# humanoid-path-planner/hpp-fcl

Hardware: AMD Instinct MI355X
Metric: narrow-phase queries/s (collision+distance) (higher is better)
Workload: dtype f32; 1 GPU; cfg3_convex32_distance_nesterov; request=distance, gather=none

## Files before the change

hpp-fcl_amd/csrc/hfcl_dev.hpp:

```cpp
#pragma once
#include <hip/hip_runtime.h>

#include <cstdint>
#include <cstring>
#include <type_traits>

#include "../../include/hppfcl_amd.h"
#include "hfcl_bvh.hpp"
#include "hfcl_bvh_shape.hpp"
#include "hfcl_epa_pool.hpp"
#include "hfcl_pair.hpp"

using namespace hfcl;

#ifndef HFCL_WPE_GJK_W2
#define HFCL_WPE_GJK_W2 2
#endif
#ifndef HFCL_WPE_GJK
#define HFCL_WPE_GJK 3
#endif
#ifndef HFCL_WPE_GJK64
#define HFCL_WPE_GJK64 2
#endif
#ifndef HFCL_WPE_PRIM
#define HFCL_WPE_PRIM 2
#endif
#ifndef HFCL_WPE_EPA32
#define HFCL_WPE_EPA32 2
#endif
#ifndef HFCL_WPE_EPA64
#define HFCL_WPE_EPA64 1
#endif
#ifndef HFCL_WPE_BVH
#define HFCL_WPE_BVH 1
#endif

enum { B_CLOSED = 0, B_PRIM = 1, B_CC = 2, B_PC = 3, B_CP = 4, B_BVH = 5, B_UNSUPPORTED = 6, B_LARGE = 7, B_BVHSHAPE = 8, B_TRI = 9, B_COUNT = 10 };
constexpr int B_CURVED0 = B_COUNT + 4;
constexpr int CTR_SHAPE_TICKET = 2 * B_COUNT + 4, CTR_SHAPE_DEFER = 2 * B_COUNT + 5;
constexpr int CTR_DIST_SUSP = 2 * B_COUNT + 6;
constexpr int CTR_SHAPE_DIST_SUSP = 2 * B_COUNT + 7;
constexpr int CTR_DIST_TICKET = 2 * B_COUNT + 8;
constexpr int CTR_SHAPE_DIST_TICKET = 2 * B_COUNT + 9;
constexpr int CTR_EPA_CC_OVER = 2 * B_COUNT + 10;
constexpr int CTR_SHAPE_FINISH_OVER = 2 * B_COUNT + 11;
constexpr int CTR_SHAPE_DEFER_MARK = 2 * B_COUNT + 13;
constexpr int CTR_DIST_RERUN = 2 * B_COUNT + 14, CTR_SHAPE_DIST_RERUN = 2 * B_COUNT + 15;
constexpr int N_COUNTERS = 2 * B_COUNT + 16;
constexpr int EPA_POOL_CTR0 = (N_COUNTERS + EPA_POOL_STRIDE_WORDS - 1) / EPA_POOL_STRIDE_WORDS * EPA_POOL_STRIDE_WORDS;
constexpr int N_COUNTER_WORDS = EPA_POOL_CTR0 + EPA_POOL_K * EPA_POOL_STRIDE_WORDS;

constexpr int K_CONVEX_LARGE = 21;

__host__ __device__ inline int bucket_of(int k1, int k2, bool distance_mode = false) {
  if (distance_mode && (k1 == K_TRIANGLE || k2 == K_TRIANGLE)) return B_UNSUPPORTED;
  const bool large = (k1 == K_CONVEX_LARGE) || (k2 == K_CONVEX_LARGE);
  if (k1 == K_CONVEX_LARGE) k1 = K_CONVEX;
  if (k2 == K_CONVEX_LARGE) k2 = K_CONVEX;
  if ((k1 == K_BVH) != (k2 == K_BVH)) {
    const int o = (k1 == K_BVH) ? k2 : k1;
    return (kind_is_prim(o) || o == K_CONVEX || kind_is_flat(o)) ? B_BVHSHAPE : B_UNSUPPORTED;
  }
  if ((k1 == K_TRIANGLE || k2 == K_TRIANGLE) && !kind_is_flat(k1) && !kind_is_flat(k2)) {
    const int o = (k1 == K_TRIANGLE) ? k2 : k1;
    return (o == K_TRIANGLE || kind_is_prim(o) || o == K_CONVEX) ? B_TRI : B_UNSUPPORTED;
  }
  const int c = pair_class(k1, k2);
  if (large && c == CLS_CONVEX) return B_LARGE;
  if (c == CLS_CLOSED) return B_CLOSED;
  if (c == CLS_PRIM_GJK) return B_PRIM;
  if (c == CLS_BVH) return B_BVH;
  if (c == CLS_CONVEX) {
    if (k1 == K_CONVEX && k2 == K_CONVEX) return B_CC;
    return (k1 == K_CONVEX) ? B_CP : B_PC;
  }
  return B_UNSUPPORTED;
}

template <typename T>
struct NbrEntry;
template <> struct alignas(16) NbrEntry<float> { float x, y, z; uint32_t id; };
template <> struct alignas(32) NbrEntry<double> { double x, y, z; uint32_t id; uint32_t pad_; };

template <typename T>
struct LibView {
  const DShape<T>* shapes;
  const T* verts;
  const uint8_t* kinds;
  uint32_t n_shapes;
  const uint32_t* graph_base;
  const uint32_t* graph_off;
  const NbrEntry<T>* graph_ent;
  uint32_t climb_min;
};
static constexpr uint32_t HFCL_NO_GRAPH = 0xFFFFFFFFu;
#ifndef HFCL_CLIMB_MIN
#define HFCL_CLIMB_MIN 512u
#endif
static constexpr int HFCL_WARM_STARTS = 14;
template <typename T>
struct HullGraph {
  const uint32_t* off;
  const NbrEntry<T>* ent;
};
template <typename T>
__device__ __forceinline__ HullGraph<T> hull_graph(const LibView<T>& lib, uint32_t shape_id, uint32_t num_points) {
  HullGraph<T> g{nullptr, nullptr};
  if (lib.graph_base == nullptr || num_points < lib.climb_min) return g;
  const uint32_t base = lib.graph_base[shape_id];
  if (base == HFCL_NO_GRAPH) return g;
  g.off = lib.graph_off + base;
  g.ent = lib.graph_ent;
  return g;
}

template <typename T> struct IO;
template <> struct IO<double> {
  const double* tf1;
  const double* tf2;
  hfcl_result* out;
  const hfcl_guess* gin;
  hfcl_guess* gout;
};
template <> struct IO<float> {
  const float* tf1;
  const float* tf2;
  hfcl_result_f32* out;
  const hfcl_guess* gin;
  hfcl_guess* gout;
};

template <typename T> using EpaItem = EpaSeed<T>;

struct Work {
  const uint32_t* shape1;
  const uint32_t* shape2;
  uint32_t n;
  uint32_t* lists;
  uint32_t* counts;
  void* epa_queue;
  void* epa_queue2;
  void* epa_v0;
  void* epa_resume;
  uint32_t resume_cap;
  void* shape_defer;
  uint32_t shape_defer_cap;
  uint32_t* shape_finish_over;
  void* shape_oq;
  void* epa_ready;
  void* epa_ready_g;
  uint32_t* epa_cc_over;
  uint32_t cc_resume_base, cc_resume_cap;
};
__host__ __device__ inline bool curved_pair(int k1, int k2) {
  return k1 == K_ELLIPSOID || k1 == K_CONE || k1 == K_CYLINDER || k2 == K_ELLIPSOID || k2 == K_CONE || k2 == K_CYLINDER;
}
struct BucketList {
  const uint32_t* base;
  uint32_t n, c0, cnt;
  __device__ __forceinline__ uint32_t operator[](uint32_t i) const { return i < c0 ? base[i] : base[n - 1u - (i - c0)]; }
};
__device__ __forceinline__ BucketList bucket_list(const Work& wk, int b) {
  const uint32_t c0 = wk.counts[b];
  return BucketList{wk.lists + size_t(b) * wk.n, wk.n, c0, c0 + wk.counts[B_CURVED0 + b]};
}
constexpr int32_t EPA_RESUME_FLAG = 0x100;
constexpr int32_t EPA_RESUME_SMALL = 0x200;

__device__ __forceinline__ Pose<double> load_pose(const double* base, uint32_t i) { return pose_from_abi<double>(base + 12 * size_t(i)); }
__device__ __forceinline__ void put_record(hfcl_result* dst, const hfcl_result& r) { *dst = r; }
__device__ __forceinline__ Pose<float> load_pose(const float* base, uint32_t i) { return pose_from_quat<float>(base + 7 * size_t(i)); }

__device__ __forceinline__ void store_record(const IO<double>& io, uint32_t pair, const PairOut<double>& o, bool contact,
                                             int nc) {
  hfcl_result r;
  r.distance = o.distance;
  r.normal[0] = o.normal.x; r.normal[1] = o.normal.y; r.normal[2] = o.normal.z;
  r.p1[0] = o.p1.x; r.p1[1] = o.p1.y; r.p1[2] = o.p1.z;
  r.p2[0] = o.p2.x; r.p2[1] = o.p2.y; r.p2[2] = o.p2.z;
  r.b1 = -1;
  r.b2 = -1;
  r.status = pack_status(o.gjk_status, o.epa_status, contact, o.gjk_iters, o.epa_iters);
  r.num_contacts = nc;
  put_record(&io.out[pair], r);
}
__device__ __forceinline__ void store_record(const IO<float>& io, uint32_t pair, const PairOut<float>& o, bool contact,
                                             int) {
  hfcl_result_f32 r;
  r.distance = o.distance;
  r.p1[0] = o.p1.x; r.p1[1] = o.p1.y; r.p1[2] = o.p1.z;
  r.p2[0] = o.p2.x; r.p2[1] = o.p2.y; r.p2[2] = o.p2.z;
  r.normal[0] = o.normal.x; r.normal[1] = o.normal.y; r.normal[2] = o.normal.z;
  r.status = pack_status(o.gjk_status, o.epa_status, contact, o.gjk_iters, o.epa_iters);
  io.out[pair] = r;
}
template <typename T>
__device__ __forceinline__ void write_out(const IO<T>& io, const QParams<T>& q, uint32_t pair, PairOut<T> o) {
  int nc;
  const bool contact = apply_query_semantics(q, o, nc);
  store_record(io, pair, o, contact, nc);
}

__device__ __forceinline__ void store_bvh_record(const IO<double>& io, uint32_t pair, const PairOut<double>& o, uint32_t nc,
                                                 int b1, int b2, bool overflow) {
  hfcl_result r;
  r.distance = o.distance;
  r.normal[0] = o.normal.x; r.normal[1] = o.normal.y; r.normal[2] = o.normal.z;
  r.p1[0] = o.p1.x; r.p1[1] = o.p1.y; r.p1[2] = o.p1.z;
  r.p2[0] = o.p2.x; r.p2[1] = o.p2.y; r.p2[2] = o.p2.z;
  r.b1 = b1;
  r.b2 = b2;
  r.status = (nc ? 128u : 0u) | (overflow ? 0xC0000000u : 0u);
  r.num_contacts = int(nc & 0x7FFFFFFFu);
  io.out[pair] = r;
}
__device__ __forceinline__ void store_bvh_record(const IO<float>& io, uint32_t pair, const PairOut<float>& o, uint32_t nc,
                                                 int, int, bool overflow) {
  hfcl_result_f32 r;
  r.distance = o.distance;
  r.p1[0] = o.p1.x; r.p1[1] = o.p1.y; r.p1[2] = o.p1.z;
  r.p2[0] = o.p2.x; r.p2[1] = o.p2.y; r.p2[2] = o.p2.z;
  r.normal[0] = o.normal.x; r.normal[1] = o.normal.y; r.normal[2] = o.normal.z;
  r.status = (nc ? 128u : 0u) | (overflow ? 0xC0000000u : 0u);
  io.out[pair] = r;
}

__device__ __forceinline__ void store_witness(const IO<double>& io, uint32_t pair, const V3<double>& p1, const V3<double>& p2, const V3<double>& n) {
  hfcl_result* r = &io.out[pair];
  r->normal[0] = n.x; r->normal[1] = n.y; r->normal[2] = n.z;
  r->p1[0] = p1.x; r->p1[1] = p1.y; r->p1[2] = p1.z;
  r->p2[0] = p2.x; r->p2[1] = p2.y; r->p2[2] = p2.z;
}
__device__ __forceinline__ void store_witness(const IO<float>& io, uint32_t pair, const V3<float>& p1, const V3<float>& p2, const V3<float>& n) {
  hfcl_result_f32* r = &io.out[pair];
  r->p1[0] = p1.x; r->p1[1] = p1.y; r->p1[2] = p1.z;
  r->p2[0] = p2.x; r->p2[1] = p2.y; r->p2[2] = p2.z;
  r->normal[0] = n.x; r->normal[1] = n.y; r->normal[2] = n.z;
}
template <typename T>
__device__ __forceinline__ void load_witness(const IO<T>& io, uint32_t pair, V3<T>& p1, V3<T>& p2, V3<T>& n) {
  const auto* r = &io.out[pair];
  n = mk<T>(T(r->normal[0]), T(r->normal[1]), T(r->normal[2]));
  p1 = mk<T>(T(r->p1[0]), T(r->p1[1]), T(r->p1[2]));
  p2 = mk<T>(T(r->p2[0]), T(r->p2[1]), T(r->p2[2]));
}
__device__ __forceinline__ void store_bvh_record_head(const IO<double>& io, uint32_t pair, double distance, uint32_t nc, int b1, int b2, bool overflow) {
  hfcl_result* r = &io.out[pair];
  r->distance = distance;
  r->b1 = b1;
  r->b2 = b2;
  r->status = (nc ? 128u : 0u) | (overflow ? 0xC0000000u : 0u);
  r->num_contacts = int(nc & 0x7FFFFFFFu);
}
__device__ __forceinline__ void store_bvh_record_head(const IO<float>& io, uint32_t pair, float distance, uint32_t nc, int, int, bool overflow) {
  hfcl_result_f32* r = &io.out[pair];
  r->distance = distance;
  r->status = (nc ? 128u : 0u) | (overflow ? 0xC0000000u : 0u);
}

template <typename T>
__device__ __forceinline__ void write_guess(const IO<T>&, uint32_t, const V3<T>&, int, int) {}
template <>
__device__ __forceinline__ void write_guess<double>(const IO<double>& io, uint32_t pair, const V3<double>& g, int h0, int h1) {
  if (io.gout) {
    hfcl_guess r;
    r.gjk_guess[0] = g.x; r.gjk_guess[1] = g.y; r.gjk_guess[2] = g.z;
    r.support_guess[0] = h0;
    r.support_guess[1] = h1;
    io.gout[pair] = r;
  }
}

template <typename T>
__device__ __forceinline__ V3<T> initial_guess(const IO<T>& io, const QParams<T>& q, uint32_t pair) {
  if (q.guess_mode == HFCL_GUESS_CACHED || q.guess_mode == HFCL_GUESS_BOUNDING_VOLUME)
    return mk<T>(q.guess[0], q.guess[1], q.guess[2]);
  return mk<T>(T(1), T(0), T(0));
}
template <>
__device__ __forceinline__ V3<double> initial_guess<double>(const IO<double>& io, const QParams<double>& q, uint32_t pair) {
  if (q.guess_mode == HFCL_GUESS_CACHED) {
    if (io.gin) return mk<double>(io.gin[pair].gjk_guess[0], io.gin[pair].gjk_guess[1], io.gin[pair].gjk_guess[2]);
    return mk<double>(q.guess[0], q.guess[1], q.guess[2]);
  }
  if (q.guess_mode == HFCL_GUESS_BOUNDING_VOLUME) return mk<double>(q.guess[0], q.guess[1], q.guess[2]);
  return mk<double>(1.0, 0.0, 0.0);
}
template <int CTRL, class X>
__device__ __forceinline__ X dpp_move(X v) {
  static_assert(sizeof(X) % 4 == 0, "32-bit words");
  int w[sizeof(X) / 4];
  __builtin_memcpy(w, &v, sizeof(X));
#pragma unroll
  for (int i = 0; i < int(sizeof(X) / 4); ++i) w[i] = __builtin_amdgcn_update_dpp(w[i], w[i], CTRL, 0xF, 0xF, false);
  X r;
  __builtin_memcpy(&r, w, sizeof(X));
  return r;
}
template <int W, int M, class X>
__device__ __forceinline__ X group_exchange(X v) {
  static_assert(M >= 1 && M < W, "stage of a W-lane butterfly");
  if constexpr (M == 1) return dpp_move<0xB1>(v);
  else if constexpr (M == 2) return dpp_move<0x4E>(v);
  else if constexpr (M == 4) return dpp_move<0x141>(v);
  else if constexpr (M == 8) return dpp_move<0x140>(v);
  else {
    int w[sizeof(X) / 4];
    __builtin_memcpy(w, &v, sizeof(X));
#pragma unroll
    for (int i = 0; i < int(sizeof(X) / 4); ++i) w[i] = __shfl_xor(w[i], M, W);
    X r;
    __builtin_memcpy(&r, w, sizeof(X));
    return r;
  }
}

constexpr int HULL_MAX = 32;
constexpr int HULL_LARGE_MAX = 1 << 16;

template <typename T, int W>
struct HullRegs {
  static constexpr int VPL = (HULL_MAX + W - 1) / W;
  V3<T> v[VPL];

  __device__ __forceinline__ void load(const T* verts, uint32_t n, int lig) {
#pragma unroll
    for (int k = 0; k < VPL; ++k) {
      uint32_t idx = uint32_t(lig * VPL + k);
      idx = idx < n ? idx : 0u;
      const T* p = verts + 3 * size_t(idx);
      v[k] = mk<T>(p[0], p[1], p[2]);
    }
  }
  __device__ __forceinline__ V3<T> support(const V3<T>& dir, int lig, int* idx_out = nullptr) const {
    T best = dot(v[0], dir);
    int bi = lig * VPL;
#pragma unroll
    for (int k = 1; k < VPL; ++k) {
      const T d = dot(v[k], dir);
      if (d > best) {
        best = d;
        bi = lig * VPL + k;
      }
    }
    butterfly_stages<W>([&](auto stage) {
      constexpr int M = decltype(stage)::value;
      const T od = group_exchange<W, M>(best);
      const int oi = group_exchange<W, M>(bi);
      const bool take = (od > best) | ((od == best) & (oi < bi));
      best = take ? od : best;
      bi = take ? oi : bi;
    });
    const int owner = bi / VPL, slot = bi % VPL;
    V3<T> c = v[0];
#pragma unroll
    for (int k = 1; k < VPL; ++k)
      if (slot == k) c = v[k];
    if (idx_out) *idx_out = bi;
    return mk<T>(__shfl(c.x, owner, W), __shfl(c.y, owner, W), __shfl(c.z, owner, W));
  }
};
template <typename T, int W>
__device__ __forceinline__ V3<T> scan_support(const T* v, uint32_t n, const V3<T>& dir, int lig, uint32_t* idx_out = nullptr) {
  T best = -Lim<T>::max();
  uint32_t bi = 0xFFFFFFFFu;
  constexpr int UNR = 8;
  uint32_t i = uint32_t(lig);
  for (; i + uint32_t((UNR - 1) * W) < n; i += uint32_t(UNR * W)) {
    T d[UNR];
#pragma unroll
    for (int u = 0; u < UNR; ++u) {
      const T* p = v + 3 * size_t(i + uint32_t(u * W));
      d[u] = p[0] * dir.x + p[1] * dir.y + p[2] * dir.z;
    }
#pragma unroll
    for (int u = 0; u < UNR; ++u)
      if (d[u] > best) {
        best = d[u];
        bi = i + uint32_t(u * W);
      }
  }
  for (; i < n; i += W) {
    const T d = v[3 * i] * dir.x + v[3 * i + 1] * dir.y + v[3 * i + 2] * dir.z;
    if (d > best) {
      best = d;
      bi = i;
    }
  }
  butterfly_stages<W>([&](auto stage) {
    constexpr int M = decltype(stage)::value;
    const T od = group_exchange<W, M>(best);
    const uint32_t oi = group_exchange<W, M>(bi);
    const bool take = (od > best) | ((od == best) & (oi < bi));
    best = take ? od : best;
    bi = take ? oi : bi;
  });
  if (idx_out) *idx_out = bi;
  return mk<T>(v[3 * bi], v[3 * bi + 1], v[3 * bi + 2]);
}
template <typename T, int W>
__device__ __forceinline__ V3<T> climb_support(const T* v, uint32_t n, const HullGraph<T>& g, const V3<T>& dir, int lig, int& hint) {
  uint32_t cur;
  T best;
  if (hint < 0) {
    best = -Lim<T>::max();
    cur = 0;
    uint32_t bk = 0xFFFFFFFFu;
    for (int k = lig; k < HFCL_WARM_STARTS; k += W) {
      const uint32_t id = g.off[k - HFCL_WARM_STARTS];
      const T d = v[3 * size_t(id)] * dir.x + v[3 * size_t(id) + 1] * dir.y + v[3 * size_t(id) + 2] * dir.z;
      if (d > best) {
        best = d;
        cur = id;
        bk = uint32_t(k);
      }
    }
    butterfly_stages<W>([&](auto stage) {
      constexpr int M = decltype(stage)::value;
      const T od = group_exchange<W, M>(best);
      const uint32_t oc = group_exchange<W, M>(cur);
      const uint32_t ok = group_exchange<W, M>(bk);
      const bool take = (od > best) | ((od == best) & (ok < bk));
      best = take ? od : best;
      cur = take ? oc : cur;
      bk = take ? ok : bk;
    });
  } else {
    cur = uint32_t(hint);
    best = v[3 * size_t(cur)] * dir.x + v[3 * size_t(cur) + 1] * dir.y + v[3 * size_t(cur) + 2] * dir.z;
  }
  bool improved = false;
  for (;;) {
    const uint32_t b = g.off[cur], e = g.off[cur + 1];
    T mb = best;
    uint32_t mi = 0xFFFFFFFFu, mpos = 0xFFFFFFFFu;
    bool tie = false;
    for (uint32_t k = b + uint32_t(lig); k < e; k += W) {
      const NbrEntry<T> nb = g.ent[k];
      const T d = nb.x * dir.x + nb.y * dir.y + nb.z * dir.z;
      tie = tie || d == best;
      if (d > mb) {
        mb = d;
        mi = nb.id;
        mpos = k;
      }
    }
    butterfly_stages<W>([&](auto stage) {
      constexpr int M = decltype(stage)::value;
      const T od = group_exchange<W, M>(mb);
      const uint32_t oi = group_exchange<W, M>(mi);
      const uint32_t ok = group_exchange<W, M>(mpos);
      const bool take = (od > mb) | ((od == mb) & (ok < mpos));
      mb = take ? od : mb;
      mi = take ? oi : mi;
      mpos = take ? ok : mpos;
    });
    if (mi == 0xFFFFFFFFu) {
      if (!improved) {
        uint32_t any = tie ? 1u : 0u;
        butterfly_stages<W>([&](auto stage) {
          constexpr int M = decltype(stage)::value;
          any |= group_exchange<W, M>(any);
        });
        if (any) {
          uint32_t si = 0;
          const V3<T> r = scan_support<T, W>(v, n, dir, lig, &si);
          hint = int(si);
          return r;
        }
      }
      break;
    }
    improved = true;
    cur = mi;
    best = mb;
  }
  hint = int(cur);
  return mk<T>(v[3 * size_t(cur)], v[3 * size_t(cur) + 1], v[3 * size_t(cur) + 2]);
}
template <typename T, int W>
__device__ __forceinline__ V3<T> large_hull_support(const T* v, uint32_t n, const HullGraph<T>& g, const V3<T>& dir, int lig, int& hint) {
  if (g.off != nullptr) return climb_support<T, W>(v, n, g, dir, lig, hint);
  return scan_support<T, W>(v, n, dir, lig);
}
template <int W_>
struct LaneGroup {
  static constexpr int W = W_;
  static __device__ __forceinline__ int lane() { return threadIdx.x & (W_ - 1); }
  template <int M, class X> static __device__ __forceinline__ X exchange(X v) { return group_exchange<W_, M>(v); }
  static __device__ __forceinline__ void sync() {
    __builtin_amdgcn_fence(__ATOMIC_ACQ_REL, "wavefront");
    __builtin_amdgcn_wave_barrier();
  }
  static __device__ __forceinline__ uint32_t atomic_inc(uint32_t* p) { return atomicAdd(p, 1u); }
  static __device__ __forceinline__ uint64_t group_bits(bool pred) {
    const uint64_t mine = (W_ == 64 ? ~uint64_t(0) : ((uint64_t(1) << (W_ & 63)) - 1u)) << ((threadIdx.x & 63) & ~(W_ - 1));
    return __ballot(pred) & mine;
  }
  static __device__ __forceinline__ uint64_t ballot(bool pred) { return group_bits(pred) >> ((threadIdx.x & 63) & ~(W_ - 1)); }
  static __device__ __forceinline__ void count(bool pred, int& below, int& total) {
    const uint64_t b = group_bits(pred);
    below = int(__builtin_amdgcn_mbcnt_hi(uint32_t(b >> 32), __builtin_amdgcn_mbcnt_lo(uint32_t(b), 0u)));
    total = __popcll(b);
  }
};

#ifndef HFCL_EPA_FAST_CAP
#define HFCL_EPA_FAST_CAP 17
#endif
constexpr int EPA_FAST_CAP = HFCL_EPA_FAST_CAP;
#ifndef HFCL_EPA_FAST_CAP64
#define HFCL_EPA_FAST_CAP64 29
#endif
#ifndef HFCL_EPA_SMALL_CAP64
#define HFCL_EPA_SMALL_CAP64 13
#endif
template <typename T> constexpr int epa_fast_cap = sizeof(T) == 4 ? EPA_FAST_CAP : HFCL_EPA_FAST_CAP64;
template <typename T> constexpr int epa_small_cap = sizeof(T) == 4 ? EPA_FAST_CAP : HFCL_EPA_SMALL_CAP64;
template <typename T> constexpr size_t epa_resume_stride = sizeof(EpaSaved<T, epa_fast_cap<T>>);
#ifndef HFCL_EPA_WE
#define HFCL_EPA_WE 8
#endif
constexpr int EPA_WE = HFCL_EPA_WE;
#ifndef HFCL_EPA_WE2
#define HFCL_EPA_WE2 16
#endif
constexpr int EPA_WE2 = HFCL_EPA_WE2;
#ifndef HFCL_EPA_WE2_64
#define HFCL_EPA_WE2_64 32
#endif
template <typename T> constexpr int epa_we2 = sizeof(T) == 4 ? HFCL_EPA_WE2 : HFCL_EPA_WE2_64;
#ifndef HFCL_EPA_CC_RESUME_WE
#define HFCL_EPA_CC_RESUME_WE 32
#endif

struct DMesh {
  uint32_t node_off, vert_off, tri_off, n_nodes;
};
template <typename T>
struct BvhView {
  const DNode<T>* nodes;
  const DNodeF* fnodes;
  const DRss<T>* rss;
  const DNodeD<T>* dnodes;
  const T* verts;
  const uint32_t* tris;
  const DMesh* meshes;
  uint32_t n_meshes;
};
struct BvhParams {
  uint32_t num_max_contacts;
  hfcl_contact* contacts;
  uint32_t contacts_cap;
  uint32_t* contacts_count;
};

struct BvhTask {
  uint32_t pair;
  uint32_t parent;
  uint32_t entry;
  uint32_t order;
};
enum { BVH_SUM_SUSPENDED = 1u, BVH_SUM_OVERFLOW = 2u };
template <typename T>
struct BvhSum {
  T dlb, rec_dist;
  T cand_val;
  V3<T> np1, np2, nn;
  int32_t fb1, fb2;
  uint32_t ncontacts, first_child, n_child, flags;
  uint32_t contact_order, parent, order, pad_;
};
#ifndef HFCL_KEEP_AB_FORMS
#define HFCL_KEEP_AB_FORMS 0
#endif
enum { BVH_CTR_TASKS = 0, BVH_CTR_SUSPENDED = 1, BVH_CTR_LEVEL0 = 2 , BVH_CTR_CUT = 15 , BVH_CTR_WORDS = 16 };
constexpr int BVH_STACK_WALK = 48;
constexpr int WALK_K = 16;
constexpr int WALK_ROUNDS = 4;
enum { WALK_OVER = 1u, WALK_BUDGET = 2u, WALK_LOST = 4u , WALK_VOID = 8u  };
template <typename T>
struct WalkRec {
  uint32_t pair, sp, n_leaf, flags;
  uint32_t first_item, pad_[3];
  T dlb, rec_dist, cand_val;
  T pre[WALK_K + 1];
  uint32_t leaf1[WALK_K], leaf2[WALK_K];
  uint32_t stack[BVH_STACK_WALK];
};
struct WalkArgs {
  void* recs;
  uint32_t* items;
  void* res;
  uint32_t* ctr;
  uint32_t* list_in;
  uint32_t* list_out;
  uint32_t* redo;
  uint32_t* perm;
  uint32_t* hist;
  uint32_t round, k, budget, last;
  uint32_t item_cap, list_stride;
};
struct BvhSplit {
  BvhTask* tasks;
  void* sums;
  uint32_t* suspended;
  uint32_t* ctr;
  uint32_t cap, n_queries;
  uint32_t budget;
  uint32_t budget0;
  uint32_t level, n_levels;
  uint32_t can_suspend;
  uint32_t leaf_cost;
  uint32_t coop;
  uint32_t coop_grid;
  uint32_t cut_ticks;
  uint32_t cut_cap;
  uint32_t cut_task_cap;
  uint32_t* cut_words;
  void* cut_vals;
  WalkArgs walk;
  uint32_t walk_rounds, walk_k[WALK_ROUNDS], walk_budget[WALK_ROUNDS];
  uint32_t coop_range;
  uint32_t* order;
};
enum { WALK_CTR_SNAP = 3, WALK_CTR_TICKET_EARLY = 4 };
constexpr int COOP_CHUNK = 16;


#ifndef HFCL_BVH_BUDGET
#define HFCL_BVH_BUDGET 0
#endif
#ifndef HFCL_BVH_BUDGET0
#define HFCL_BVH_BUDGET0 HFCL_BVH_BUDGET
#endif
struct BvhSpill {
  void* slab;
  uint32_t cap;
  uint32_t max_blocks;
  uint32_t wide;
  void* susp;
  uint32_t* susp_count;
  uint32_t budget;
  uint32_t pool;
  uint32_t* pool_ticket;
  uint32_t pool_leaf_min, pool_starve, pool_part_min;
  uint32_t* rerun_count;
  uint32_t rerun_all;
};
constexpr int BVH_MAX_LEVELS = 12;
#ifndef HFCL_BVH_LEVELS
#define HFCL_BVH_LEVELS 6
#endif

#ifndef HFCL_BVH_STACK
#define HFCL_BVH_STACK 48
#endif
constexpr int BVH_STACK = HFCL_BVH_STACK;

template <bool WIDE> struct BvhEntry;
template <> struct BvhEntry<false> {
  typedef uint32_t E;
  static constexpr int STACK = BVH_STACK;
  static __device__ __forceinline__ E pack(uint32_t b1, uint32_t b2) { return b1 | (b2 << 16); }
  static __device__ __forceinline__ uint32_t first(E e) { return e & 0xFFFFu; }
  static __device__ __forceinline__ uint32_t second(E e) { return e >> 16; }
};
template <> struct BvhEntry<true> {
  typedef uint64_t E;
  static constexpr int STACK = BVH_STACK / 2;
  static __device__ __forceinline__ E pack(uint32_t b1, uint32_t b2) { return uint64_t(b1) | (uint64_t(b2) << 32); }
  static __device__ __forceinline__ uint32_t first(E e) { return uint32_t(e); }
  static __device__ __forceinline__ uint32_t second(E e) { return uint32_t(e >> 32); }
};

#ifndef HFCL_BVH_STACK_FILT
#define HFCL_BVH_STACK_FILT 26
#endif
constexpr int BVH_STACK_FILT = HFCL_BVH_STACK_FILT;
constexpr int BVH_BLOCK = 128;
#ifndef HFCL_BVH_REFILL_MIN
#define HFCL_BVH_REFILL_MIN 8
#endif
constexpr int BVH_REFILL_MIN = HFCL_BVH_REFILL_MIN;

constexpr int CLS_BLOCK = 1024;
constexpr int LARGE_W = 16;
constexpr int BS_W = 16;
constexpr int BS_STACK = 128;
constexpr int BVHD_STACK = 40;
constexpr int BVHD_BLOCK = 64;
__device__ __forceinline__ float chain_up(double d) { return __double2float_ru(d); }
__device__ __forceinline__ float chain_up(float d) { return d; }
template <typename T>
struct ShapeDistSusp {
  uint32_t pair, sp;
  int32_t fb1, pad_;
  T mind;
  uint32_t entry[BVHD_STACK];
  T bound[BVHD_STACK];
};
template <typename T>
struct DistSusp {
  uint32_t pair, sp;
  int32_t fb1, fb2;
  T mind;
  V3<T> np1, np2;
  uint32_t entry[BVHD_STACK];
  T bound[BVHD_STACK];
};

struct PSlot {
  uint32_t s;
};
__device__ __forceinline__ PSlot psel(bool c, const PSlot& a, const PSlot& b) { return PSlot{c ? a.s : b.s}; }
template <typename T, int NT>
struct W0Lds {
  typedef PSlot P;
  static constexpr int WORDS = 4 * 3 * NT;
  T* lane;
  template <class G>
  __device__ __forceinline__ P put(const G& g, const V3<T>& w0) const {
    uint32_t used = g.rank > 0 ? 1u << (g.s0.p.s & 3u) : 0u;
    used |= g.rank > 1 ? 1u << (g.s1.p.s & 3u) : 0u;
    used |= g.rank > 2 ? 1u << (g.s2.p.s & 3u) : 0u;
    const uint32_t s = uint32_t(__builtin_ctz(~used)) & 3u;
    lane[(3 * s + 0) * NT] = w0.x;
    lane[(3 * s + 1) * NT] = w0.y;
    lane[(3 * s + 2) * NT] = w0.z;
    return P{s};
  }
  __device__ __forceinline__ V3<T> get(const P& p) const {
    const uint32_t s = p.s & 3u;
    return mk<T>(lane[(3 * s + 0) * NT], lane[(3 * s + 1) * NT], lane[(3 * s + 2) * NT]);
  }
};
#ifndef HFCL_GJK_W0_LDS
#define HFCL_GJK_W0_LDS 1
#endif
```

hpp-fcl_amd/csrc/hfcl_k_gjk.hip:

```cpp
#include "hfcl_dev.hpp"
#include "hfcl_launch.hpp"

#ifndef HFCL_UNIT_PRECISION
#define HFCL_UNIT_PRECISION 0
#endif
#define HFCL_UNIT_F32 (HFCL_UNIT_PRECISION != 64)
#define HFCL_UNIT_F64 (HFCL_UNIT_PRECISION != 32)

#if HFCL_UNIT_F64
__global__ void __launch_bounds__(CLS_BLOCK) k_classify(Work wk, const uint8_t* kinds, uint32_t n_shapes, bool distance_mode) {
  constexpr int PER_THREAD = 8;
  constexpr uint32_t CHUNK = CLS_BLOCK * PER_THREAD;
  __shared__ uint32_t s_count[2 * B_COUNT];
  __shared__ uint32_t s_base[2 * B_COUNT];
  for (uint32_t start = blockIdx.x * CHUNK; start < wk.n; start += gridDim.x * CHUNK) {
    if (threadIdx.x < 2 * B_COUNT) s_count[threadIdx.x] = 0;
    __syncthreads();
    int bk[PER_THREAD];
    uint32_t rk[PER_THREAD];
#pragma unroll
    for (int k = 0; k < PER_THREAD; ++k) {
      const uint32_t i = start + k * CLS_BLOCK + threadIdx.x;
      bk[k] = -1;
      rk[k] = 0;
      if (i < wk.n) {
        const uint32_t s1 = wk.shape1[i], s2 = wk.shape2[i];
        if (s1 < n_shapes && s2 < n_shapes) {
          const int k1 = kinds[s1], k2 = kinds[s2];
          bk[k] = bucket_of(k1, k2, distance_mode);
          if ((bk[k] == B_PRIM || bk[k] == B_PC || bk[k] == B_CP) && curved_pair(k1, k2)) bk[k] += B_COUNT;
        } else {
          bk[k] = B_UNSUPPORTED;
        }
      }
      unsigned long long todo = __ballot(bk[k] >= 0);
      const int lane = threadIdx.x & 63;
      while (todo) {
        const int leader = __ffsll((long long)todo) - 1;
        const int c = __shfl(bk[k], leader, 64);
        const unsigned long long m = __ballot(bk[k] == c);
        uint32_t base = 0;
        if (lane == leader) base = atomicAdd(&s_count[c], (uint32_t)__popcll(m));
        base = __shfl(base, leader, 64);
        if (bk[k] == c) rk[k] = base + (uint32_t)__popcll(m & ((1ull << lane) - 1ull));
        todo &= ~m;
      }
    }
    __syncthreads();
    if (threadIdx.x < 2 * B_COUNT) {
      const uint32_t c = s_count[threadIdx.x];
      const int counter = threadIdx.x < B_COUNT ? int(threadIdx.x) : B_CURVED0 + int(threadIdx.x) - B_COUNT;
      s_base[threadIdx.x] = c ? atomicAdd(&wk.counts[counter], c) : 0u;
    }
    __syncthreads();
#pragma unroll
    for (int k = 0; k < PER_THREAD; ++k) {
      if (bk[k] < 0) continue;
      const uint32_t slot = s_base[bk[k]] + rk[k], id = start + k * CLS_BLOCK + threadIdx.x;
      if (bk[k] < B_COUNT)
        wk.lists[size_t(bk[k]) * wk.n + slot] = id;
      else
        wk.lists[size_t(bk[k] - B_COUNT) * wk.n + (wk.n - 1u - slot)] = id;
    }
    __syncthreads();
  }
}

#endif
template <typename T>
__global__ void __launch_bounds__(256) k_unsupported(Work wk, IO<T> io, int bucket) {
  const uint32_t cnt = wk.counts[bucket];
  for (uint32_t it = blockIdx.x * blockDim.x + threadIdx.x; it < cnt; it += gridDim.x * blockDim.x) {
    const uint32_t pair = wk.lists[size_t(bucket) * wk.n + it];
    auto r = io.out[pair];
    memset(&r, 0, sizeof(r));
    r.status = 0x80000000u;
    io.out[pair] = r;
  }
}

template <typename T>
__global__ void __launch_bounds__(256) k_closed(Work wk, LibView<T> lib, IO<T> io, QParams<T> q) {
  const uint32_t cnt = wk.counts[B_CLOSED];
  for (uint32_t it = blockIdx.x * blockDim.x + threadIdx.x; it < cnt; it += gridDim.x * blockDim.x) {
    const uint32_t pair = wk.lists[size_t(B_CLOSED) * wk.n + it];
    const DShape<T> a = lib.shapes[wk.shape1[pair]], b = lib.shapes[wk.shape2[pair]];
    const Pose<T> tf1 = load_pose(io.tf1, pair), tf2 = load_pose(io.tf2, pair);
    PairOut<T> o;
    o.distance = closed_form_distance(a, tf1, b, tf2, lib.verts, o.p1, o.p2, o.normal);
    o.gjk_status = GJK_DID_NOT_RUN;
    o.epa_status = EPA_DID_NOT_RUN;
    o.gjk_iters = o.epa_iters = 0;
    write_out<T>(io, q, pair, o);
    write_guess<T>(io, pair, initial_guess<T>(io, q, pair), 0, 0);
  }
}

#if HFCL_UNIT_F64
typedef double hfcl_d2 __attribute__((ext_vector_type(2)));
#ifndef HFCL_WPE_CLOSED
#define HFCL_WPE_CLOSED 2
#endif
__global__ void __launch_bounds__(256) __attribute__((amdgpu_waves_per_eu(HFCL_WPE_CLOSED, 8))) k_closed_staged(Work wk, LibView<double> lib, IO<double> io, QParams<double> q) {
  constexpr int NB = 256, PIECES = 6;
  __shared__ uint32_t s_pair[NB];
  __shared__ hfcl_d2 s_a[NB * PIECES];
  __shared__ hfcl_d2 s_b[NB * PIECES];
  static_assert(sizeof(hfcl_result) == 96, "record = 6 pieces");
  const uint32_t cnt = wk.counts[B_CLOSED];
  const uint32_t t = threadIdx.x;
  for (uint32_t base = blockIdx.x * NB; base < cnt; base += gridDim.x * NB) {
    const uint32_t nvalid = min(uint32_t(NB), cnt - base);
    s_pair[t] = wk.lists[size_t(B_CLOSED) * wk.n + base + (t < nvalid ? t : 0u)];
    __syncthreads();
#pragma unroll
    for (int j = 0; j < PIECES; ++j) {
      const uint32_t c = t + NB * j, p = c / PIECES, part = c % PIECES;
      const size_t pr = s_pair[p];
      s_a[c] = reinterpret_cast<const hfcl_d2*>(io.tf1 + 12 * pr)[part];
      s_b[c] = reinterpret_cast<const hfcl_d2*>(io.tf2 + 12 * pr)[part];
    }
    const uint32_t pair = s_pair[t];
    const DShape<double> a = lib.shapes[wk.shape1[pair]], b = lib.shapes[wk.shape2[pair]];
    __syncthreads();
    const Pose<double> tf1 = pose_from_abi<double>(reinterpret_cast<const double*>(s_a + PIECES * t));
    const Pose<double> tf2 = pose_from_abi<double>(reinterpret_cast<const double*>(s_b + PIECES * t));
    PairOut<double> o;
    o.distance = closed_form_distance(a, tf1, b, tf2, lib.verts, o.p1, o.p2, o.normal);
    o.gjk_status = GJK_DID_NOT_RUN;
    o.epa_status = EPA_DID_NOT_RUN;
    o.gjk_iters = o.epa_iters = 0;
    __syncthreads();
    IO<double> lio = io;
    lio.out = reinterpret_cast<hfcl_result*>(s_a);
    write_out<double>(lio, q, t, o);
    if (t < nvalid) write_guess<double>(io, pair, initial_guess<double>(io, q, pair), 0, 0);
    __syncthreads();
#pragma unroll
    for (int j = 0; j < PIECES; ++j) {
      const uint32_t c = t + NB * j, p = c / PIECES, part = c % PIECES;
      if (p < nvalid) reinterpret_cast<hfcl_d2*>(io.out + s_pair[p])[part] = s_a[c];
    }
    __syncthreads();
  }
}

#endif
template <typename T, class P, class PS>
__device__ __forceinline__ void finish_gjk(const Gjk<T, P>& g, const Work& wk, const IO<T>& io, const QParams<T>& q,
                                           uint32_t pair, const Pose<T>& tf1, T r0, T r1, const V3<T>& guess0,
                                           bool writer, const PS& ps, bool full_tier = false, bool cc_queue = false) {
  PairOut<T> o;
  EpaSeed<T> seed;
  const bool to_epa = gjk_finish(g, q, tf1, r0, r1, guess0, o, seed, ps);
  if (!writer) return;
  if (to_epa) {
    seed.pair = pair;
    if (cc_queue) {
#ifdef HFCL_EXPERIMENT_NO_QUEUE_ATOMIC
      const uint32_t slot = pair;
#else
      const uint32_t slot = atomicAdd(&wk.counts[B_COUNT + 3], 1u);
#endif
      reinterpret_cast<EpaSeed<T>*>(wk.epa_queue)[wk.n - 1u - slot] = seed;
    } else {
      const uint32_t slot = atomicAdd(&wk.counts[full_tier ? B_COUNT + 1 : B_COUNT], 1u);
      reinterpret_cast<EpaSeed<T>*>(full_tier ? wk.epa_queue2 : wk.epa_queue)[slot] = seed;
    }
  } else {
    write_out<T>(io, q, pair, o);
    write_guess<T>(io, pair, o.cached_guess, 0, 0);
  }
}

#if HFCL_GJK_W0_LDS
template <typename T, int NT> using GjkW0 = W0Lds<T, NT>;
#define HFCL_GJK_W0_SLAB(T, NT, name)          \
  __shared__ T name##_slab[W0Lds<T, NT>::WORDS]; \
  const W0Lds<T, NT> name{name##_slab + threadIdx.x}
#else
template <typename T, int NT> using GjkW0 = W0Regs<T>;
#define HFCL_GJK_W0_SLAB(T, NT, name) const W0Regs<T> name = W0Regs<T>()
#endif

template <typename T, bool BVG>
__global__ void __launch_bounds__(256) __attribute__((amdgpu_waves_per_eu(HFCL_WPE_PRIM, 8))) k_gjk_prim(Work wk, LibView<T> lib, IO<T> io, QParams<T> q) {
  HFCL_GJK_W0_SLAB(T, 256, ps);
  const BucketList list = bucket_list(wk, B_PRIM);
  for (uint32_t it = blockIdx.x * blockDim.x + threadIdx.x; it < list.cnt; it += gridDim.x * blockDim.x) {
    const uint32_t pair = list[it];
    const DShape<T> a = lib.shapes[wk.shape1[pair]], b = lib.shapes[wk.shape2[pair]];
    const Pose<T> tf1 = load_pose(io.tf1, pair), tf2 = load_pose(io.tf2, pair);
    SerialSupport<T> sup;
    sup.a = a;
    sup.b = b;
    sup.va = sup.vb = nullptr;
    sup.md = make_mdiff(tf1, tf2);
    const T r0 = swept_radius(a), r1 = swept_radius(b);
    const V3<T> guess0 = initial_guess<T>(io, q, pair);
    Gjk<T, typename GjkW0<T, 256>::P> g;
    if constexpr (BVG)
      gjk_run(g, q.gjk, start_guess(q, a, b, sup.md, guess0), r0 + r1, false, sup, ps);
    else
      gjk_run(g, q.gjk, guess0, r0 + r1, false, sup, ps);
    finish_gjk<T>(g, wk, io, q, pair, tf1, r0, r1, guess0, true, ps, false, sizeof(T) == 8 && curved_pair(a.kind, b.kind));
  }
}
#ifndef HFCL_HULL_LDS_BATCH
#define HFCL_HULL_LDS_BATCH 4
#endif
template <typename T, int W, int NT>
struct HullLds {
  static constexpr int VPL = (HULL_MAX + W - 1) / W;
  static constexpr int WORDS = VPL * 3 * NT;
  T* lane;
  __device__ __forceinline__ void load(const T* verts, uint32_t n, int lig) {
#pragma unroll
    for (int k = 0; k < VPL; ++k) {
      uint32_t idx = uint32_t(lig * VPL + k);
      idx = idx < n ? idx : 0u;
      const T* p = verts + 3 * size_t(idx);
      lane[(3 * k + 0) * NT] = p[0];
      lane[(3 * k + 1) * NT] = p[1];
      lane[(3 * k + 2) * NT] = p[2];
    }
  }
  __device__ __forceinline__ V3<T> support(const V3<T>& dir, int lig) const {
#if HFCL_HULL_LDS_BATCH
    constexpr int B = HFCL_HULL_LDS_BATCH;
    T best = T(0);
    int bi = lig * VPL;
#pragma unroll
    for (int k0 = 0; k0 < VPL; k0 += B) {
      T vx[B], vy[B], vz[B];
#pragma unroll
      for (int j = 0; j < B; ++j) {
        vx[j] = lane[(3 * (k0 + j) + 0) * NT];
        vy[j] = lane[(3 * (k0 + j) + 1) * NT];
        vz[j] = lane[(3 * (k0 + j) + 2) * NT];
      }
      __builtin_amdgcn_sched_barrier(0);
#pragma unroll
      for (int j = 0; j < B; ++j) {
        const T d = vx[j] * dir.x + vy[j] * dir.y + vz[j] * dir.z;
        if (k0 + j == 0) {
          best = d;
        } else if (d > best) {
          best = d;
          bi = lig * VPL + k0 + j;
        }
      }
      __builtin_amdgcn_sched_barrier(0);
    }
#else
    T best = lane[0] * dir.x + lane[NT] * dir.y + lane[2 * NT] * dir.z;
    int bi = lig * VPL;
#pragma unroll
    for (int k = 1; k < VPL; ++k) {
      const T d = lane[(3 * k + 0) * NT] * dir.x + lane[(3 * k + 1) * NT] * dir.y + lane[(3 * k + 2) * NT] * dir.z;
      if (d > best) {
        best = d;
        bi = lig * VPL + k;
      }
    }
#endif
    butterfly_stages<W>([&](auto stage) {
      constexpr int M = decltype(stage)::value;
      const T od = group_exchange<W, M>(best);
      const int oi = group_exchange<W, M>(bi);
      const bool take = (od > best) | ((od == best) & (oi < bi));
      best = take ? od : best;
      bi = take ? oi : bi;
    });
    const int owner = bi / VPL, slot = bi % VPL;
    const T cx = lane[(3 * slot + 0) * NT], cy = lane[(3 * slot + 1) * NT], cz = lane[(3 * slot + 2) * NT];
    return mk<T>(__shfl(cx, owner, W), __shfl(cy, owner, W), __shfl(cz, owner, W));
  }
};
#ifndef HFCL_GJK_HULLB_LDS
#define HFCL_GJK_HULLB_LDS 1
#endif
template <typename T, int W, int M> constexpr bool hull_b_in_lds = HFCL_GJK_HULLB_LDS && M == 0 && W <= 4 && (HULL_MAX / W) * sizeof(T) <= 64;

template <typename T, int W, int M, int NT>
struct CvxSupport {
  DShape<T> a, b;
  HullRegs<T, W> h0;
  typename std::conditional<hull_b_in_lds<T, W, M>, HullLds<T, W, NT>, HullRegs<T, W>>::type h1;
  MDiff<T> md;
  int lig;
  __device__ __forceinline__ void eval(const V3<T>& dir, V3<T>& w, V3<T>& w0) const {
    if (M == 1)
      w0 = prim_support(a, dir);
    else
      w0 = h0.support(dir, lig);
    const V3<T> d1 = md.identity ? -dir : -tmul(md.oR1, dir);
    V3<T> s1;
    if (M == 2)
      s1 = prim_support(b, d1);
    else
      s1 = h1.support(d1, lig);
    s1 = md.identity ? s1 : (mul(md.oR1, s1) + md.ot1);
    w = w0 - s1;
  }
  __device__ __forceinline__ void operator()(const V3<T>& dir, V3<T>& w, V3<T>& w0) const { eval(dir, w, w0); }
};

template <typename T, int W, int M, bool BVG, int NT>
__device__ __forceinline__ void gjk_cvx_body(const Work& wk, const LibView<T>& lib, const IO<T>& io, const QParams<T>& q) {
  constexpr int BUCKET = (M == 0) ? B_CC : (M == 1 ? B_PC : B_CP);
  HFCL_GJK_W0_SLAB(T, NT, ps);
  __shared__ T hull_slab[hull_b_in_lds<T, W, M> ? HullLds<T, W, NT>::WORDS : 1];
  const BucketList list = bucket_list(wk, BUCKET);
  const int lig = threadIdx.x & (W - 1);
  const uint32_t groups = (gridDim.x * blockDim.x) / W;
  for (uint32_t it = (blockIdx.x * blockDim.x + threadIdx.x) / W; it < list.cnt; it += groups) {
    const uint32_t pair = list[it];
    CvxSupport<T, W, M, NT> sup;
    if constexpr (hull_b_in_lds<T, W, M>) sup.h1.lane = hull_slab + threadIdx.x;
    sup.a = lib.shapes[wk.shape1[pair]];
    sup.b = lib.shapes[wk.shape2[pair]];
    sup.lig = lig;
    if (M != 1) sup.h0.load(lib.verts + 3 * size_t(sup.a.vertex_offset), sup.a.num_points, lig);
    if (M != 2) sup.h1.load(lib.verts + 3 * size_t(sup.b.vertex_offset), sup.b.num_points, lig);
    const Pose<T> tf1 = load_pose(io.tf1, pair), tf2 = load_pose(io.tf2, pair);
    sup.md = make_mdiff(tf1, tf2);
    const T r0 = swept_radius(sup.a), r1 = swept_radius(sup.b);
    const V3<T> guess0 = initial_guess<T>(io, q, pair);
    Gjk<T, typename GjkW0<T, NT>::P> g;
    if constexpr (BVG)
      gjk_run(g, q.gjk, start_guess(q, sup.a, sup.b, sup.md, guess0), r0 + r1, M == 0, sup, ps);
    else
      gjk_run(g, q.gjk, guess0, r0 + r1, M == 0, sup, ps);
    finish_gjk<T>(g, wk, io, q, pair, tf1, r0, r1, guess0, lig == 0, ps, false,
                  sizeof(T) == 4 ? M == 0 : (M != 0 && curved_pair(sup.a.kind, sup.b.kind)));
  }
}

template <int W, int M, bool BVG>
__global__ void __launch_bounds__(gjk_cvx_threads<float>(W, M)) __attribute__((amdgpu_waves_per_eu(W == 2 ? HFCL_WPE_GJK_W2 : HFCL_WPE_GJK, 8)))
k_gjk_cvx(Work wk, LibView<float> lib, IO<float> io, QParams<float> q) {
  gjk_cvx_body<float, W, M, BVG, gjk_cvx_threads<float>(W, M)>(wk, lib, io, q);
}
template <int W, int M, bool BVG>
__global__ void __launch_bounds__(gjk_cvx_threads<double>(W, M)) __attribute__((amdgpu_waves_per_eu(HFCL_WPE_GJK64, 8)))
k_gjk_cvx64(Work wk, LibView<double> lib, IO<double> io, QParams<double> q) {
  gjk_cvx_body<double, W, M, BVG, gjk_cvx_threads<double>(W, M)>(wk, lib, io, q);
}
template <int W, int M, bool BVG = false>
static void launch_gjk_cvx(int grid, hipStream_t st, const Work& wk, const LibView<float>& lv, const IO<float>& io, const QParams<float>& q) {
  hipLaunchKernelGGL((k_gjk_cvx<W, M, BVG>), dim3(grid), dim3(gjk_cvx_threads<float>(W, M)), 0, st, wk, lv, io, q);
}
template <int W, int M, bool BVG = false>
static void launch_gjk_cvx(int grid, hipStream_t st, const Work& wk, const LibView<double>& lv, const IO<double>& io, const QParams<double>& q) {
  hipLaunchKernelGGL((k_gjk_cvx64<W, M, BVG>), dim3(grid), dim3(gjk_cvx_threads<double>(W, M)), 0, st, wk, lv, io, q);
}
template <typename T>
struct LargeSupport {
  DShape<T> a, b;
  const T* va;
  const T* vb;
  HullGraph<T> ga, gb;
  mutable int hint0, hint1;
  MDiff<T> md;
  int lig;
  __device__ __forceinline__ V3<T> one(const DShape<T>& s, const T* v, const HullGraph<T>& g, const V3<T>& d, int& hint) const {
    return s.kind == K_CONVEX ? large_hull_support<T, LARGE_W>(v, s.num_points, g, d, lig, hint) : prim_support(s, d);
  }
  __device__ __forceinline__ void operator()(const V3<T>& dir, V3<T>& w, V3<T>& w0) const {
    w0 = one(a, va, ga, dir, hint0);
    const V3<T> d1 = md.identity ? -dir : -tmul(md.oR1, dir);
    V3<T> s1 = one(b, vb, gb, d1, hint1);
    s1 = md.identity ? s1 : (mul(md.oR1, s1) + md.ot1);
    w = w0 - s1;
  }
};

template <typename T, bool BVG>
__global__ void __launch_bounds__(256) __attribute__((amdgpu_waves_per_eu(2, 8))) k_gjk_large(Work wk, LibView<T> lib, IO<T> io, QParams<T> q) {
  HFCL_GJK_W0_SLAB(T, 256, ps);
  const uint32_t cnt = wk.counts[B_LARGE];
  const int lig = threadIdx.x & (LARGE_W - 1);
  const uint32_t groups = (gridDim.x * blockDim.x) / LARGE_W;
  for (uint32_t it = (blockIdx.x * blockDim.x + threadIdx.x) / LARGE_W; it < cnt; it += groups) {
    const uint32_t pair = wk.lists[size_t(B_LARGE) * wk.n + it];
    LargeSupport<T> sup;
    const uint32_t sid1 = wk.shape1[pair], sid2 = wk.shape2[pair];
    sup.a = lib.shapes[sid1];
    sup.b = lib.shapes[sid2];
    sup.va = lib.verts + 3 * size_t(sup.a.vertex_offset);
    sup.vb = lib.verts + 3 * size_t(sup.b.vertex_offset);
    sup.ga = sup.a.kind == K_CONVEX ? hull_graph(lib, sid1, sup.a.num_points) : HullGraph<T>{nullptr, nullptr};
    sup.gb = sup.b.kind == K_CONVEX ? hull_graph(lib, sid2, sup.b.num_points) : HullGraph<T>{nullptr, nullptr};
    sup.hint0 = sup.hint1 = -1;
    sup.lig = lig;
    const Pose<T> tf1 = load_pose(io.tf1, pair), tf2 = load_pose(io.tf2, pair);
    sup.md = make_mdiff(tf1, tf2);
    const T r0 = swept_radius(sup.a), r1 = swept_radius(sup.b);
    const V3<T> guess0 = initial_guess<T>(io, q, pair);
    Gjk<T, typename GjkW0<T, 256>::P> g;
    if constexpr (BVG)
      gjk_run(g, q.gjk, start_guess(q, sup.a, sup.b, sup.md, guess0), r0 + r1, sup.a.kind == K_CONVEX && sup.b.kind == K_CONVEX, sup, ps);
    else
      gjk_run(g, q.gjk, guess0, r0 + r1, sup.a.kind == K_CONVEX && sup.b.kind == K_CONVEX, sup, ps);
    finish_gjk<T>(g, wk, io, q, pair, tf1, r0, r1, guess0, lig == 0, ps, true);
  }
}

template <typename R>
__global__ void k_fill_skipped(R* out, uint32_t n) {
  for (uint32_t i = blockIdx.x * blockDim.x + threadIdx.x; i < n; i += gridDim.x * blockDim.x) {
    R r;
    memset(&r, 0, sizeof(r));
    r.distance = 3.402823466e+38f;
    r.status = 0x80000000u;
    out[i] = r;
  }
}
#if HFCL_UNIT_F64
template <>
__global__ void k_fill_skipped<hfcl_result>(hfcl_result* out, uint32_t n) {
  for (uint32_t i = blockIdx.x * blockDim.x + threadIdx.x; i < n; i += gridDim.x * blockDim.x) {
    hfcl_result r;
    const double x = __builtin_nan("");
    r.distance = 1.7976931348623157e+308;
    for (int k = 0; k < 3; ++k) r.normal[k] = r.p1[k] = r.p2[k] = x;
    r.b1 = r.b2 = -1;
    r.status = 0x80000000u;
    r.num_contacts = 0;
    out[i] = r;
  }
}

#endif
#if HFCL_UNIT_F64
__global__ void __launch_bounds__(256) k_expand_poses(const double* qt, double* tf, uint32_t n) {
  for (uint32_t i = blockIdx.x * blockDim.x + threadIdx.x; i < n; i += gridDim.x * blockDim.x) {
    const Pose<double> p = pose_from_quat<double, double>(qt + 7 * size_t(i));
    double* o = tf + 12 * size_t(i);
    o[0] = p.R.r0.x; o[1] = p.R.r1.x; o[2] = p.R.r2.x;
    o[3] = p.R.r0.y; o[4] = p.R.r1.y; o[5] = p.R.r2.y;
    o[6] = p.R.r0.z; o[7] = p.R.r1.z; o[8] = p.R.r2.z;
    o[9] = p.t.x; o[10] = p.t.y; o[11] = p.t.z;
  }
}
#endif
#if HFCL_UNIT_F64
void launch_expand_poses(hipStream_t st, const double* qt, double* tf, uint32_t n) {
  hipLaunchKernelGGL(k_expand_poses, dim3(1024), dim3(256), 0, st, qt, tf, n);
}
#endif

#if HFCL_UNIT_F64
void launch_classify(int grid, hipStream_t st, const Work& wk, const uint8_t* kinds, uint32_t n_shapes, bool distance_mode) {
  hipLaunchKernelGGL(k_classify, dim3(grid), dim3(CLS_BLOCK), 0, st, wk, kinds, n_shapes, distance_mode);
}
#endif
template <typename T>
void launch_unsupported(int grid, hipStream_t st, const Work& wk, const IO<T>& io, int bucket) {
  hipLaunchKernelGGL((k_unsupported<T>), dim3(grid), dim3(256), 0, st, wk, io, bucket);
}
#if HFCL_UNIT_F32
template void launch_unsupported<float>(int, hipStream_t, const Work&, const IO<float>&, int);
#endif
#if HFCL_UNIT_F64
template void launch_unsupported<double>(int, hipStream_t, const Work&, const IO<double>&, int);
#endif

template <typename T>
void launch_closed(int grid, hipStream_t st, const Work& wk, const LibView<T>& lv, const IO<T>& io, const QParams<T>& q, bool staged) {
#if HFCL_UNIT_F64
  if constexpr (sizeof(T) == 8) {
    if (staged) {
      hipLaunchKernelGGL(k_closed_staged, dim3(grid), dim3(256), 0, st, wk, lv, io, q);
      return;
    }
  }
#endif
  hipLaunchKernelGGL((k_closed<T>), dim3(grid), dim3(256), 0, st, wk, lv, io, q);
}
#if HFCL_UNIT_F32
template void launch_closed<float>(int, hipStream_t, const Work&, const LibView<float>&, const IO<float>&, const QParams<float>&, bool);
#endif
#if HFCL_UNIT_F64
template void launch_closed<double>(int, hipStream_t, const Work&, const LibView<double>&, const IO<double>&, const QParams<double>&, bool);
#endif

template <typename T>
void launch_gjk_prim(int grid, hipStream_t st, const Work& wk, const LibView<T>& lv, const IO<T>& io, const QParams<T>& q, bool bvg) {
  if (bvg)
    hipLaunchKernelGGL((k_gjk_prim<T, true>), dim3(grid), dim3(256), 0, st, wk, lv, io, q);
  else
    hipLaunchKernelGGL((k_gjk_prim<T, false>), dim3(grid), dim3(256), 0, st, wk, lv, io, q);
}
#if HFCL_UNIT_F32
template void launch_gjk_prim<float>(int, hipStream_t, const Work&, const LibView<float>&, const IO<float>&, const QParams<float>&, bool);
#endif
#if HFCL_UNIT_F64
template void launch_gjk_prim<double>(int, hipStream_t, const Work&, const LibView<double>&, const IO<double>&, const QParams<double>&, bool);
#endif

template <typename T, int M>
static void launch_gjk_cvx_m(int w, bool bvg, int grid, hipStream_t st, const Work& wk, const LibView<T>& lv, const IO<T>& io, const QParams<T>& q) {
  if (bvg) {
    if (w == 2) launch_gjk_cvx<2, M, true>(grid, st, wk, lv, io, q);
    else launch_gjk_cvx<4, M, true>(grid, st, wk, lv, io, q);
    return;
  }
  switch (w) {
    case 2: launch_gjk_cvx<2, M>(grid, st, wk, lv, io, q); break;
    case 8: launch_gjk_cvx<8, M>(grid, st, wk, lv, io, q); break;
    case 16: launch_gjk_cvx<16, M>(grid, st, wk, lv, io, q); break;
    case 32: launch_gjk_cvx<32, M>(grid, st, wk, lv, io, q); break;
    case 64: launch_gjk_cvx<64, M>(grid, st, wk, lv, io, q); break;
    default: launch_gjk_cvx<4, M>(grid, st, wk, lv, io, q); break;
  }
}
template <typename T>
void launch_gjk_cvx(int m, int w, bool bvg, int grid, hipStream_t st, const Work& wk, const LibView<T>& lv, const IO<T>& io, const QParams<T>& q) {
  if (m == 0) launch_gjk_cvx_m<T, 0>(w, bvg, grid, st, wk, lv, io, q);
  else if (m == 1) launch_gjk_cvx_m<T, 1>(w, bvg, grid, st, wk, lv, io, q);
  else launch_gjk_cvx_m<T, 2>(w, bvg, grid, st, wk, lv, io, q);
}
#if HFCL_UNIT_F32
template void launch_gjk_cvx<float>(int, int, bool, int, hipStream_t, const Work&, const LibView<float>&, const IO<float>&, const QParams<float>&);
#endif
#if HFCL_UNIT_F64
template void launch_gjk_cvx<double>(int, int, bool, int, hipStream_t, const Work&, const LibView<double>&, const IO<double>&, const QParams<double>&);
#endif

template <typename T>
void launch_gjk_large(int grid, hipStream_t st, const Work& wk, const LibView<T>& lv, const IO<T>& io, const QParams<T>& q, bool bvg) {
  if (bvg)
    hipLaunchKernelGGL((k_gjk_large<T, true>), dim3(grid), dim3(256), 0, st, wk, lv, io, q);
  else
    hipLaunchKernelGGL((k_gjk_large<T, false>), dim3(grid), dim3(256), 0, st, wk, lv, io, q);
}
#if HFCL_UNIT_F32
template void launch_gjk_large<float>(int, hipStream_t, const Work&, const LibView<float>&, const IO<float>&, const QParams<float>&, bool);
#endif
#if HFCL_UNIT_F64
template void launch_gjk_large<double>(int, hipStream_t, const Work&, const LibView<double>&, const IO<double>&, const QParams<double>&, bool);
#endif

#if HFCL_UNIT_F64
void launch_fill_skipped(hipStream_t st, hfcl_result* out, uint32_t n) {
  hipLaunchKernelGGL((k_fill_skipped<hfcl_result>), dim3(1024), dim3(256), 0, st, out, n);
}
#endif
#if HFCL_UNIT_F32
void launch_fill_skipped(hipStream_t st, hfcl_result_f32* out, uint32_t n) {
  hipLaunchKernelGGL((k_fill_skipped<hfcl_result_f32>), dim3(1024), dim3(256), 0, st, out, n);
}
#endif
```

Baseline: 643.4 million queries/s.

## Store GJK simplex support points as hull vertex indices for f32 W=2 convex pairs

```diff
diff --git a/hpp-fcl_amd/csrc/hfcl_dev.hpp b/hpp-fcl_amd/csrc/hfcl_dev.hpp
--- a/hpp-fcl_amd/csrc/hfcl_dev.hpp
+++ b/hpp-fcl_amd/csrc/hfcl_dev.hpp
@@ -15,6 +15,9 @@
 
 #ifndef HFCL_WPE_GJK_W2
 #define HFCL_WPE_GJK_W2 2
+#endif
+#ifndef HFCL_WPE_GJK_CC2
+#define HFCL_WPE_GJK_CC2 3
 #endif
 #ifndef HFCL_WPE_GJK
 #define HFCL_WPE_GJK 3
diff --git a/hpp-fcl_amd/csrc/hfcl_k_gjk.hip b/hpp-fcl_amd/csrc/hfcl_k_gjk.hip
--- a/hpp-fcl_amd/csrc/hfcl_k_gjk.hip
+++ b/hpp-fcl_amd/csrc/hfcl_k_gjk.hip
@@ -173,19 +173,35 @@
   }
 }
 
-#if HFCL_GJK_W0_LDS
-template <typename T, int NT> using GjkW0 = W0Lds<T, NT>;
-#define HFCL_GJK_W0_SLAB(T, NT, name)          \
-  __shared__ T name##_slab[W0Lds<T, NT>::WORDS]; \
-  const W0Lds<T, NT> name{name##_slab + threadIdx.x}
-#else
-template <typename T, int NT> using GjkW0 = W0Regs<T>;
-#define HFCL_GJK_W0_SLAB(T, NT, name) const W0Regs<T> name = W0Regs<T>()
-#endif
+enum { W0_REGS = 0, W0_LANE = 1, W0_GROUP = 2, W0_INDEX = 3 };
+constexpr int GJK_W0_DEFAULT = HFCL_GJK_W0_LDS ? W0_LANE : W0_REGS;
+template <typename T, int NT, int MODE, int G = 1>
+__device__ __forceinline__ auto gjk_w0() {
+  static_assert(MODE == W0_REGS || MODE == W0_LANE || MODE == W0_GROUP, "W0_INDEX is made per pair (gjk_cvx_body)");
+  if constexpr (MODE == W0_REGS) {
+    return W0Regs<T>();
+  } else {
+    constexpr int SLOTS = MODE == W0_GROUP ? NT / G : NT;
+    __shared__ T slab[W0Lds<T, SLOTS>::WORDS];
+    return W0Lds<T, SLOTS>{slab + (MODE == W0_GROUP ? threadIdx.x / G : threadIdx.x)};
+  }
+}
+template <typename T>
+struct W0Index {
+  typedef PSlot P;
+  const int* last;
+  const T* verts;
+  uint32_t n;
+  template <class G> __device__ __forceinline__ P put(const G&, const V3<T>&) const { return P{uint32_t(*last)}; }
+  __device__ __forceinline__ V3<T> get(const P& p) const {
+    const T* q = verts + 3 * size_t(p.s < n ? p.s : 0u);
+    return mk<T>(q[0], q[1], q[2]);
+  }
+};
 
 template <typename T, bool BVG>
 __global__ void __launch_bounds__(256) __attribute__((amdgpu_waves_per_eu(HFCL_WPE_PRIM, 8))) k_gjk_prim(Work wk, LibView<T> lib, IO<T> io, QParams<T> q) {
-  HFCL_GJK_W0_SLAB(T, 256, ps);
+  const auto ps = gjk_w0<T, 256, GJK_W0_DEFAULT>();
   const BucketList list = bucket_list(wk, B_PRIM);
   for (uint32_t it = blockIdx.x * blockDim.x + threadIdx.x; it < list.cnt; it += gridDim.x * blockDim.x) {
     const uint32_t pair = list[it];
@@ -198,7 +214,7 @@
     sup.md = make_mdiff(tf1, tf2);
     const T r0 = swept_radius(a), r1 = swept_radius(b);
     const V3<T> guess0 = initial_guess<T>(io, q, pair);
-    Gjk<T, typename GjkW0<T, 256>::P> g;
+    Gjk<T, typename decltype(ps)::P> g;
     if constexpr (BVG)
       gjk_run(g, q.gjk, start_guess(q, a, b, sup.md, guess0), r0 + r1, false, sup, ps);
     else
@@ -282,8 +298,9 @@
 #endif
 template <typename T, int W, int M> constexpr bool hull_b_in_lds = HFCL_GJK_HULLB_LDS && M == 0 && W <= 4 && (HULL_MAX / W) * sizeof(T) <= 64;
 
-template <typename T, int W, int M, int NT>
+template <typename T, int W, int M, int NT, bool IDX = false>
 struct CvxSupport {
+  mutable int i0;
   DShape<T> a, b;
   HullRegs<T, W> h0;
   typename std::conditional<hull_b_in_lds<T, W, M>, HullLds<T, W, NT>, HullRegs<T, W>>::type h1;
@@ -293,7 +310,7 @@
     if (M == 1)
       w0 = prim_support(a, dir);
     else
-      w0 = h0.support(dir, lig);
+      w0 = h0.support(dir, lig, IDX ? &i0 : nullptr);
     const V3<T> d1 = md.identity ? -dir : -tmul(md.oR1, dir);
     V3<T> s1;
     if (M == 2)
@@ -306,17 +323,25 @@
   __device__ __forceinline__ void operator()(const V3<T>& dir, V3<T>& w, V3<T>& w0) const { eval(dir, w, w0); }
 };
 
+#ifndef HFCL_GJK_CC2_W0
+#define HFCL_GJK_CC2_W0 3
+#endif
+template <typename T, int W, int M> constexpr int gjk_cvx_w0 = (sizeof(T) == 4 && W == 2 && M == 0) ? HFCL_GJK_CC2_W0 : GJK_W0_DEFAULT;
+static_assert(HFCL_GJK_CC2_W0 >= W0_REGS && HFCL_GJK_CC2_W0 <= W0_INDEX, "HFCL_GJK_CC2_W0: one of W0_REGS, W0_LANE, W0_GROUP, W0_INDEX");
+
 template <typename T, int W, int M, bool BVG, int NT>
 __device__ __forceinline__ void gjk_cvx_body(const Work& wk, const LibView<T>& lib, const IO<T>& io, const QParams<T>& q) {
   constexpr int BUCKET = (M == 0) ? B_CC : (M == 1 ? B_PC : B_CP);
-  HFCL_GJK_W0_SLAB(T, NT, ps);
+  constexpr bool IDX = gjk_cvx_w0<T, W, M> == W0_INDEX;
+  static_assert(!IDX || M != 1, "W0_INDEX: shape 0 is a register-resident hull");
+  const auto ps0 = gjk_w0<T, NT, IDX ? W0_REGS : gjk_cvx_w0<T, W, M>, W>();
   __shared__ T hull_slab[hull_b_in_lds<T, W, M> ? HullLds<T, W, NT>::WORDS : 1];
   const BucketList list = bucket_list(wk, BUCKET);
   const int lig = threadIdx.x & (W - 1);
   const uint32_t groups = (gridDim.x * blockDim.x) / W;
   for (uint32_t it = (blockIdx.x * blockDim.x + threadIdx.x) / W; it < list.cnt; it += groups) {
     const uint32_t pair = list[it];
-    CvxSupport<T, W, M, NT> sup;
+    CvxSupport<T, W, M, NT, IDX> sup;
     if constexpr (hull_b_in_lds<T, W, M>) sup.h1.lane = hull_slab + threadIdx.x;
     sup.a = lib.shapes[wk.shape1[pair]];
     sup.b = lib.shapes[wk.shape2[pair]];
@@ -327,7 +352,13 @@
     sup.md = make_mdiff(tf1, tf2);
     const T r0 = swept_radius(sup.a), r1 = swept_radius(sup.b);
     const V3<T> guess0 = initial_guess<T>(io, q, pair);
-    Gjk<T, typename GjkW0<T, NT>::P> g;
+    const auto ps = [&] {
+      if constexpr (IDX)
+        return W0Index<T>{&sup.i0, lib.verts + 3 * size_t(sup.a.vertex_offset), sup.a.num_points};
+      else
+        return ps0;
+    }();
+    Gjk<T, typename decltype(ps)::P> g;
     if constexpr (BVG)
       gjk_run(g, q.gjk, start_guess(q, sup.a, sup.b, sup.md, guess0), r0 + r1, M == 0, sup, ps);
     else
@@ -338,7 +369,7 @@
 }
 
 template <int W, int M, bool BVG>
-__global__ void __launch_bounds__(gjk_cvx_threads<float>(W, M)) __attribute__((amdgpu_waves_per_eu(W == 2 ? HFCL_WPE_GJK_W2 : HFCL_WPE_GJK, 8)))
+__global__ void __launch_bounds__(gjk_cvx_threads<float>(W, M)) __attribute__((amdgpu_waves_per_eu(W == 2 ? (M == 0 ? HFCL_WPE_GJK_CC2 : HFCL_WPE_GJK_W2) : HFCL_WPE_GJK, 8)))
 k_gjk_cvx(Work wk, LibView<float> lib, IO<float> io, QParams<float> q) {
   gjk_cvx_body<float, W, M, BVG, gjk_cvx_threads<float>(W, M)>(wk, lib, io, q);
 }
@@ -378,7 +409,7 @@
 
 template <typename T, bool BVG>
 __global__ void __launch_bounds__(256) __attribute__((amdgpu_waves_per_eu(2, 8))) k_gjk_large(Work wk, LibView<T> lib, IO<T> io, QParams<T> q) {
-  HFCL_GJK_W0_SLAB(T, 256, ps);
+  const auto ps = gjk_w0<T, 256, GJK_W0_DEFAULT>();
   const uint32_t cnt = wk.counts[B_LARGE];
   const int lig = threadIdx.x & (LARGE_W - 1);
   const uint32_t groups = (gridDim.x * blockDim.x) / LARGE_W;
@@ -398,7 +429,7 @@
     sup.md = make_mdiff(tf1, tf2);
     const T r0 = swept_radius(sup.a), r1 = swept_radius(sup.b);
     const V3<T> guess0 = initial_guess<T>(io, q, pair);
-    Gjk<T, typename GjkW0<T, 256>::P> g;
+    Gjk<T, typename decltype(ps)::P> g;
     if constexpr (BVG)
       gjk_run(g, q.gjk, start_guess(q, sup.a, sup.b, sup.md, guess0), r0 + r1, sup.a.kind == K_CONVEX && sup.b.kind == K_CONVEX, sup, ps);
     else
```

New measurement: 711.4 million queries/s, median of 6. 10.6% higher.
